# dselivanov/rsparse

Hardware: AMD Instinct MI355X
Metric: als_iterations_per_sec (higher is better)
Workload: dtype f32 (Gram products of rows > 512 / <= 32 non-zeros as 2 x fp16 / 3 x bf16 split terms of the fp32 operands, fp32 accumulate; everything else fp32); 1 GPU; WRMF implicit ALS, CG(3), synthetic 10000000x1000000, 500155883 nnz, rank 128, lambda 0.1; survey_config=3, feedback=implicit, n_items=1000000, nnz=500155883, rank=128, solver=conjugate_gradient, cg_steps=3, parallelism=rows sharded x1, factors replicated

## Files before the change

### rsparse_amd/csrc/wrmf_cgq.hip

```cpp
#include <algorithm>

#include "wrmf_internal.h"
#include "wrmf_device.h"

namespace rsparse_hip {
namespace {

using namespace dev;

constexpr int kGvFirstMinCapq = 16;
constexpr int kStreamPrefixQ = 4;
constexpr int kIdxPrefetchMaxWpr = 2;

constexpr int kMaxSavedSweeps = 4;

template <int KP>
struct QG {
  static constexpr int RPN = KP / 16;
  static constexpr int VW = RPN >= 4 ? 4 : RPN;
  static constexpr int NV = RPN / VW;
  __device__ static __forceinline__ int elem(int i, int r) { return (r / VW) * (16 * VW) + i * VW + (r % VW); }
};

template <int VW>
struct Piece;
template <>
struct Piece<4> { using type = float4; };
template <>
struct Piece<2> { using type = float2; };

__device__ __forceinline__ float groups_reduce_scatter4(const float a0, const float a1, const float a2, const float a3) {
  const auto s01 = __builtin_amdgcn_permlane16_swap(__float_as_uint(a0), __float_as_uint(a1), false, false);
  const float c = __uint_as_float(s01[0]) + __uint_as_float(s01[1]);
  const auto s23 = __builtin_amdgcn_permlane16_swap(__float_as_uint(a2), __float_as_uint(a3), false, false);
  const float d = __uint_as_float(s23[0]) + __uint_as_float(s23[1]);
  const auto t = __builtin_amdgcn_permlane32_swap(__float_as_uint(c), __float_as_uint(d), false, false);
  return __uint_as_float(t[0]) + __uint_as_float(t[1]);
}
template <int KP, int CAPQ, int WAVES, int WPR, int STREAM, bool IMPLICIT, int DMF = 0>
struct QSmem {
  static constexpr size_t gram_floats = (IMPLICIT && DMF != 1) ? (size_t)KP * KP : 0;
  static constexpr size_t vec_floats = IMPLICIT ? (size_t)WAVES * KP : 0;
  static constexpr size_t red_floats = WPR > 1 ? (size_t)2 * WAVES * KP + 2 * WAVES : 0;
  static constexpr bool cv_lds = !STREAM && CAPQ * (KP / 16) > 128;
  static constexpr bool wideq = !STREAM && CAPQ * (KP / 16) > 160;
  static constexpr size_t tsv_floats = (STREAM && !IMPLICIT) ? 0 : (size_t)WAVES * (cv_lds ? 3 : 2) * CAPQ * 4;
  static constexpr size_t pre_floats = STREAM ? (size_t)WAVES * kStreamPrefixQ * 4 * KP : 0;
  static constexpr int dmf_ps = KP + 8, dmf_os = KP + 4;
  static constexpr size_t dmf_floats = DMF ? (size_t)WAVES * dmf_ps + (size_t)WAVES * dmf_os : 0;
  static constexpr size_t pfx_floats =
      (!STREAM && WPR > kIdxPrefetchMaxWpr && (CAPQ == 16 || CAPQ == 20 || CAPQ == 24)) ? (size_t)WAVES * 2 * CAPQ * 4 : 0;
  static constexpr size_t wl_floats = cv_lds ? (size_t)WAVES * 2 : 0;
  static constexpr size_t xs_floats = cv_lds ? (size_t)WAVES * KP : 0;
  static constexpr size_t bytes =
      (gram_floats + vec_floats + red_floats + tsv_floats + pre_floats + dmf_floats + pfx_floats + wl_floats + xs_floats) * 4 + 16;
};

constexpr int kLastFull = 0, kLastDotsInLoop = 1, kLastDotsBehind = 2;
struct LastStepChoice { int kp, capq, waves, wpr, stream; bool implicit; int dmf; bool gb, kfull; int form; };
constexpr LastStepChoice kLastStepChoices[] = {
    {64, 32, 4, 1, 0, true, 0, true, false, kLastFull},
    {64, 16, 4, 1, 0, true, 0, true, true, kLastFull},
    {64, 32, 4, 1, 0, true, 0, false, true, kLastFull},
    {64, 16, 4, 1, 0, true, 0, false, false, kLastFull},
    {64, 16, 4, 1, 0, false, 0, false, true, kLastFull},
    {128, 16, 8, 8, 0, true, 0, true, true, kLastFull},
    {128, 16, 8, 8, 0, true, 0, true, false, kLastFull},
    {128, 16, 4, 2, 0, true, 0, true, true, kLastFull},
    {128, 16, 4, 1, 0, true, 2, true, true, kLastFull},
    {128, 16, 8, 8, 0, true, 0, false, false, kLastFull},
    {32, 8, 4, 1, 0, false, 0, false, true, kLastDotsBehind},
    {64, 32, 4, 2, 0, true, 0, true, false, kLastDotsBehind},
    {64, 32, 4, 2, 0, true, 0, false, false, kLastDotsBehind},
    {128, 16, 4, 4, 0, true, 0, true, false, kLastDotsBehind},
    {128, 16, 4, 2, 0, true, 0, true, false, kLastDotsBehind},
    {128, 24, 4, 4, 0, true, 0, false, true, kLastDotsBehind},
    {128, 24, 4, 4, 0, true, 0, false, false, kLastDotsBehind},
    {128, 20, 4, 4, 0, true, 0, false, true, kLastDotsBehind},
    {128, 20, 4, 4, 0, true, 0, false, false, kLastDotsBehind},
    {128, 16, 4, 4, 0, true, 0, false, false, kLastDotsBehind},
    {128, 16, 4, 2, 0, true, 0, false, false, kLastDotsBehind},
    {128, 16, 4, 1, 0, true, 2, false, false, kLastDotsBehind},
    {128, 20, 4, 4, 0, false, 0, false, true, kLastDotsBehind},
};
constexpr int last_step_form(int KP, int CAPQ, int WAVES, int WPR, int STREAM, bool IMPLICIT, int DMF, bool GB, bool KFULL) {
  for (const LastStepChoice& c : kLastStepChoices)
    if (c.kp == KP && c.capq == CAPQ && c.waves == WAVES && c.wpr == WPR && c.stream == STREAM && c.implicit == IMPLICIT &&
        c.dmf == DMF && c.gb == GB && c.kfull == KFULL)
      return c.form;
  return kLastDotsInLoop;
}

template <int KP, int CAPQ, int WAVES, int WPR, int STREAM, bool IMPLICIT, int DMF = 0, bool GB = false, bool KFULL = false>
__global__ __launch_bounds__(WAVES * 64, 2) void als_cgq_kernel(AlsArgs a, const int32_t* __restrict__ rows, int n_rows,
                                                             int rows_per_team, size_t loss_slot0) {
  using G_ = QG<KP>;
  constexpr int RPN = G_::RPN, VW = G_::VW, NV = G_::NV, CAP = CAPQ * 4, TEAMS = WAVES / WPR;
  using piece_t = typename Piece<VW>::type;
  using SM = QSmem<KP, CAPQ, WAVES, WPR, STREAM, IMPLICIT, DMF>;
  static_assert(WAVES % WPR == 0, "teams must tile the workgroup");
  constexpr bool GRS = RPN == 8 && VW == 4;
  auto groups_all_reduce8 = [](float(&a8)[RPN]) {
    if constexpr (RPN == 8) {
      const float r0 = groups_reduce_scatter4(a8[0], a8[1], a8[2], a8[3]);
      const float r1 = groups_reduce_scatter4(a8[4], a8[5], a8[6], a8[7]);
      float g0[4], g1[4];
      rows_to_all<4>(r0, g0);
      rows_to_all<4>(r1, g1);
#pragma unroll
      for (int e = 0; e < 4; e++) a8[e] = g0[e], a8[4 + e] = g1[e];
    }
  };
  static_assert(!DMF || (IMPLICIT && KP == 128 && WAVES == 4 && WPR == 1 && STREAM == 0), "DMF geometry");
  static_assert(DMF != 1 || CAPQ == 8, "register-resident G terms: only the 8-quad kernel has the 64 registers");
  static_assert(!GB || IMPLICIT, "the global bias of explicit feedback is removed from the data (R/model_WRMF.R:278-282)");
  const float gbias = GB ? a.gbias : 0.f, ltgt = GB ? a.loss_tgt_const : 1.f;
  extern __shared__ __attribute__((aligned(16))) char smem[];
  float* sG = reinterpret_cast<float*>(smem);
  float* sVec = sG + SM::gram_floats;
  float* sRed = sVec + SM::vec_floats;
  float* sRedL = sRed + (WPR > 1 ? 2 * WAVES * KP : 0);
  float* sTsv = sVec + SM::vec_floats + SM::red_floats;
  float* sPre = sTsv + SM::tsv_floats;
  float* sPfx = sPre + SM::pre_floats;
  _Float16* sPh = reinterpret_cast<_Float16*>(sPre + SM::pre_floats);
  _Float16* sPl = sPh + WAVES * SM::dmf_ps;
  float* sOut = reinterpret_cast<float*>(sPl + WAVES * SM::dmf_ps);

  const int tid = threadIdx.x, lane = tid & 63, wv = rfl(tid >> 6);
  const int g = lane >> 4, i = lane & 15;
  const int team = wv / WPR, tw = wv % WPR;
  const int k = KFULL ? KP : a.k;
  if constexpr (IMPLICIT && DMF == 0) {
    constexpr int GU = (KP * KP) % (8 * WAVES * 64) == 0 ? 8 : ((KP * KP) % (2 * WAVES * 64) == 0 ? 2 : 1);
    static_assert((KP * KP) % (GU * WAVES * 64) == 0, "the Gramian copy walks whole batches");
    for (int e0 = tid; e0 < KP * KP; e0 += GU * WAVES * 64) {
      float gv[GU];
#pragma unroll
      for (int u = 0; u < GU; u++) {
        const int e = e0 + u * WAVES * 64, r = e / KP, c = e % KP;
        gv[u] = a.XtX[(size_t)min(r, k - 1) * k + min(c, k - 1)];
      }
#pragma unroll
      for (int u = 0; u < GU; u++) {
        const int e = e0 + u * WAVES * 64, r = e / KP, c = e % KP;
        sG[e] = (r < k && c < k) ? gv[u] : 0.f;
      }
    }
  }
  for (int e = tid; e < (int)(SM::vec_floats + SM::red_floats + SM::tsv_floats); e += WAVES * 64) sVec[e] = 0.f;
  __syncthreads();

  constexpr int NRES = (IMPLICIT && CAPQ == 8 && WPR == 1 && !STREAM && KP == 128 && !DMF) ? 2 : 0;
  piece_t gres[NRES > 0 ? NRES : 1][4][NV];
  if constexpr (NRES > 0) {
#pragma unroll
    for (int rs = 0; rs < NRES; rs++)
#pragma unroll
      for (int u = 0; u < 4; u++)
#pragma unroll
        for (int b = 0; b < NV; b++)
          gres[rs][u][b] = *reinterpret_cast<const piece_t*>(sG + (4 * (g + 4 * rs) + u) * KP + b * 16 * VW + i * VW);
  }
  f16x8 gAh[DMF == 1 ? 2 : 1][DMF == 1 ? 4 : 1], gAl[DMF == 1 ? 2 : 1][DMF == 1 ? 4 : 1];
  char* sGf = reinterpret_cast<char*>(sG) + (size_t)wv * 16 * 1024;
  float ginv = 1.f;
  if constexpr (DMF) {
    const int m = lane & 15, kb = lane >> 4;
    float gmax = 0.f;
#pragma unroll
    for (int t = 0; t < 2; t++)
#pragma unroll
      for (int ks = 0; ks < 4; ks++)
#pragma unroll
        for (int e = 0; e < 8; e++) {
          const int r = 32 * wv + 16 * t + m, c = 32 * ks + 8 * kb + e;
          {
            const float gv = a.XtX[(size_t)min(r, k - 1) * k + min(c, k - 1)];
            gmax = fmaxf(gmax, fabsf(gv) * ((r < k && c < k) ? 1.f : 0.f));
          }
        }
    for (int o = 32; o > 0; o >>= 1) gmax = fmaxf(gmax, __shfl_xor(gmax, o));
    const int ge = fp16_scale_exp(gmax);
    const float gs = __uint_as_float((unsigned)ge << 23);
    ginv = __uint_as_float((unsigned)(254 - ge) << 23);
#pragma unroll
    for (int t = 0; t < 2; t++)
#pragma unroll
      for (int ks = 0; ks < 4; ks++) {
        unsigned hi[4], lo[4];
#pragma unroll
        for (int e = 0; e < 8; e += 2) {
          const int r = 32 * wv + 16 * t + m, c = 32 * ks + 8 * kb + e;
          const float g0v = a.XtX[(size_t)min(r, k - 1) * k + min(c, k - 1)];
          const float g0 = g0v * ((r < k && c < k) ? 1.f : 0.f);
          const float g1v = a.XtX[(size_t)min(r, k - 1) * k + min(c + 1, k - 1)];
          const float g1 = g1v * ((r < k && c + 1 < k) ? 1.f : 0.f);
          split_f16(g0 * gs, g1 * gs, hi[e / 2], lo[e / 2]);
        }
        const uint4 h4 = {hi[0], hi[1], hi[2], hi[3]}, l4 = {lo[0], lo[1], lo[2], lo[3]};
        if constexpr (DMF == 1) {
          gAh[t][ks] = __builtin_bit_cast(f16x8, h4);
          gAl[t][ks] = __builtin_bit_cast(f16x8, l4);
        } else {
          *reinterpret_cast<uint4*>(sGf + ((t * 4 + ks) * 2 + 0) * 1024 + lane * 16) = h4;
          *reinterpret_cast<uint4*>(sGf + ((t * 4 + ks) * 2 + 1) * 1024 + lane * 16) = l4;
        }
      }
    if constexpr (DMF == 2) wave_sync();
  }
  float* vec = sVec + wv * KP;
  constexpr bool CVLDS = SM::cv_lds;
  constexpr bool WIDEQ = SM::wideq;
  float* tacc = sTsv + wv * (CVLDS ? 3 : 2) * CAP;
  float* tcur = tacc + CAP;
  float* csv = tcur + CAP;
  int buf = 0;
  double wloss = 0.0;
  double* wl_lds = reinterpret_cast<double*>(sPfx + SM::pfx_floats) + wv;
  if (CVLDS && lane == 0) *wl_lds = 0.0;
  float* xs = sPfx + SM::pfx_floats + SM::wl_floats + wv * KP;
  int pf_id = 0, pf_cnt = -1;
  float pf_c = 0.f;
  const int team_global = blockIdx.x * TEAMS + team;
  const int total_teams = gridDim.x * TEAMS;

  auto row_index = [&](int itn) { return team_global + itn * total_teams; };
  int row_c = 0, p1_c = 0, p2_c = 0, row_n = 0;
  if (rows_per_team > 0 && row_index(0) < n_rows) {
    row_c = rows[row_index(0)];
    p1_c = a.col_ptrs[row_c];
    p2_c = a.col_ptrs[row_c + 1];
  }
  if (rows_per_team > 1 && row_index(1) < n_rows) row_n = rows[row_index(1)];
  for (int it = 0; it < rows_per_team; ++it) {
    const int ri = row_index(it);
    const bool have = ri < n_rows;
    if (WPR == 1 && !DMF && !have) break;
    const int row = have ? rfl(row_c) : 0;
    const int p1 = have ? rfl(p1_c) : 0;
    const int p2 = have ? rfl(p2_c) : 0;
    constexpr bool META_LATE = WIDEQ && !KFULL;
#define RSP_ADVANCE_META()                                                      \
    {                                                                           \
      int p1_n = 0, p2_n = 0, row_nn = 0;                                       \
      if (it + 1 < rows_per_team && row_index(it + 1) < n_rows) {               \
        p1_n = a.col_ptrs[row_n];                                               \
        p2_n = a.col_ptrs[row_n + 1];                                           \
      }                                                                         \
      if (it + 2 < rows_per_team && row_index(it + 2) < n_rows) row_nn = rows[row_index(it + 2)]; \
      row_c = row_n;                                                            \
      p1_c = p1_n;                                                              \
      p2_c = p2_n;                                                              \
      row_n = row_nn;                                                           \
    }
    if constexpr (!META_LATE) RSP_ADVANCE_META()
    const int cnt = p2 - p1;
    float* yrow = a.Y + (size_t)row * k;
    if (!GB && WPR == 1 && cnt <= 0) {
      if (!DMF || have)
        for (int e = lane; e < k; e += 64) yrow[e] = 0.f;
      if constexpr (!DMF) continue;
    }
    constexpr int PQ = STREAM ? kStreamPrefixQ : 0, PCAP = PQ * 4, PTEAM = PCAP * WPR;
    const int pre = STREAM ? min(cnt, PTEAM) : 0;
    const int pw = STREAM ? max(0, min(PCAP, pre - tw * PCAP)) : 0;
    const int nchunks = (cnt - pre + CAP - 1) / CAP;
    constexpr bool resident = STREAM == 0;
    const float lam_use =
        IMPLICIT ? 0.f : (float)(a.lambda_loss * (a.dynamic_lambda ? (double)(float)cnt : 1.0));

    float* tscr = nullptr;
    float alph[kMaxSavedSweeps];
#pragma unroll
    for (int s2 = 0; s2 < kMaxSavedSweeps; s2++) alph[s2] = 0.f;
    if constexpr (STREAM == 1) {
      if (a.tscr && have && a.cg_steps <= kMaxSavedSweeps) tscr = a.tscr + a.stream_off[ri];
    }

    float xt[CAPQ][RPN];
    float cv[CVLDS ? 1 : CAPQ];
    constexpr int NSL = (CAP + 63) / 64;
    float cl[CVLDS ? 1 : NSL];
#pragma unroll
    for (int s2 = 0; s2 < (CVLDS ? 1 : NSL); s2++) cl[s2] = 0.f;
    auto csv_fill = [&](auto&& conf_of, const int n) {
      const int ln = opaque_lane<WIDEQ>(lane);
#pragma unroll
      for (int s2 = 0; s2 < NSL; s2++) {
        const int sl = ln + 64 * s2;
        if (s2 == 0 || sl < CAP) csv[(sl & 3) * CAPQ + (sl >> 2)] = sl < n ? conf_of(sl) : 0.f;
      }
    };
    int ccnt = 0;

    constexpr bool ZPAD = STREAM == 0;
    constexpr bool TSAVE = STREAM == 0;
    constexpr bool GVFIRST = STREAM == 0 && CAPQ >= kGvFirstMinCapq;
    constexpr bool IDXPF = CAP <= 64 && ((STREAM == 0 && WPR <= kIdxPrefetchMaxWpr) || (STREAM == 1 && IMPLICIT));
    constexpr bool DMAPF = KFULL && !IDXPF && SM::pfx_floats > 0;
    int* pfxI = reinterpret_cast<int*>(sPfx) + wv * 2 * CAP;
    float* pfxC = sPfx + wv * 2 * CAP + CAP;
    auto dma_slot = [&](const int j0, const int n) {
      const int j = j0 + min(lane, n - 1);
      dma4(a.row_idx + j, lds_addr(pfxI));
      dma4(a.vals + j, lds_addr(pfxC));
      if constexpr (CAP > 64) {
        if (lane < CAP - 64) {
          const int j2 = j0 + min(lane + 64, n - 1);
          dma4(a.row_idx + j2, lds_addr(pfxI + 64));
          dma4(a.vals + j2, lds_addr(pfxC + 64));
        }
      }
    };
    int pf_pos = -1;
#define RSP_SLOT_IN(q, n) (SM::wideq ? g < (n) - 4 * (q) : 4 * (q) + g < (n))
#define RSP_SLOT_J(q, n) max(SM::wideq ? min(g, (n) - 1 - 4 * (q)) + 4 * (q) : min(4 * (q) + g, (n) - 1), 0)
    auto gather_q = [&](auto nq_tag, const int base, const int n, const bool from_pf = false) {
      constexpr int NQG = decltype(nq_tag)::value;
      int id[NQG > 0 ? NQG : 1];
      if constexpr (DMAPF) {
        if (!from_pf && n > 0) {
          dma_slot(base, n);
          wait_vm<0>();
        }
        wave_sync();
#pragma unroll
        for (int q = 0; q < NQG; q++) {
          const int j = RSP_SLOT_J(q, n);
          id[q] = pfxI[j];
          if constexpr (!CVLDS) cv[q] = (!ZPAD || RSP_SLOT_IN(q, n)) ? pfxC[j] : 0.f;
        }
        if constexpr (CVLDS) {
          csv_fill([&](int sl) { return pfxC[sl]; }, n);
        } else if constexpr (TSAVE) {
          const int lo = opaque_lane<true>(lane);
#pragma unroll
          for (int s2 = 0; s2 < NSL; s2++) cl[s2] = lane + 64 * s2 < n ? pfxC[min(lo + 64 * s2, CAP - 1)] : 0.f;
        }
        wave_sync();
      } else if (IDXPF && from_pf) {
        int* xi = reinterpret_cast<int*>(tacc);
        wave_sync();
        xi[lane & (CAP - 1)] = pf_id;
        tcur[lane & (CAP - 1)] = pf_c;
        wave_sync();
#pragma unroll
        for (int q = 0; q < NQG; q++) {
          const int j = RSP_SLOT_J(q, n);
          id[q] = xi[j];
          if constexpr (!CVLDS) cv[q] = (!ZPAD || RSP_SLOT_IN(q, n)) ? tcur[j] : 0.f;
        }
        if constexpr (TSAVE) cl[0] = lane < n ? pf_c : 0.f;
        wave_sync();
      } else {
#pragma unroll
        for (int q = 0; q < NQG; q++) {
          const int j = RSP_SLOT_J(q, n);
          id[q] = a.row_idx[base + j];
          if constexpr (!CVLDS) {
            const float c = a.vals[base + j];
            cv[q] = (!ZPAD || RSP_SLOT_IN(q, n)) ? c : 0.f;
          }
        }
        if constexpr (CVLDS) {
          wave_sync();
          csv_fill([&](int sl) { return a.vals[base + sl]; }, n);
          wave_sync();
        } else if constexpr (TSAVE) {
#pragma unroll
          for (int s2 = 0; s2 < NSL; s2++) cl[s2] = lane + 64 * s2 < n ? a.vals[base + lane + 64 * s2] : 0.f;
        }
      }
      const int ig = (SM::wideq && !KFULL) ? (opaque_lane<true>(lane) & 15) : i;
#pragma unroll
      for (int q = 0; q < NQG; q++) {
        const float* src = (!ZPAD || RSP_SLOT_IN(q, n)) ? a.X + (size_t)id[q] * k : a.zero_row;
#pragma unroll
        for (int b = 0; b < NV; b++) {
          const int off = b * 16 * VW + ig * VW;
          if constexpr (KFULL) {
            const piece_t pc = *reinterpret_cast<const piece_t*>(src + off);
            const float* pf = reinterpret_cast<const float*>(&pc);
#pragma unroll
            for (int c = 0; c < VW; c++) xt[q][b * VW + c] = pf[c];
          } else {
            const piece_t pc = *reinterpret_cast<const piece_t*>(src + min(off, k - VW));
            const float* pf = reinterpret_cast<const float*>(&pc);
#pragma unroll
            for (int c = 0; c < VW; c++) xt[q][b * VW + c] = off < k ? pf[c] : 0.f;
          }
        }
      }
    };
#undef RSP_SLOT_IN
#undef RSP_SLOT_J
    auto gather = [&](const int base, const int n, const bool from_pf = false) {
      gather_q(std::integral_constant<int, CAPQ>{}, base, n, from_pf);
    };
    float* pre_lds = sPre + (size_t)wv * PQ * 4 * KP + g * KP;
    auto prefix_chunk = [&](const bool first) {
      if constexpr (PQ > 0) {
        const int base = p1 + tw * PCAP;
        if (first) {
          gather_q(std::integral_constant<int, PQ>{}, base, pw);
#pragma unroll
          for (int q = 0; q < PQ; q++)
#pragma unroll
            for (int b = 0; b < NV; b++) {
              piece_t pc;
              float* pf = reinterpret_cast<float*>(&pc);
#pragma unroll
              for (int c = 0; c < VW; c++) pf[c] = xt[q][b * VW + c];
              *reinterpret_cast<piece_t*>(pre_lds + q * 4 * KP + b * 16 * VW + i * VW) = pc;
            }
        } else {
#pragma unroll
          for (int q = 0; q < PQ; q++) cv[q] = a.vals[base + min(4 * q + g, pw - 1)];
#pragma unroll
          for (int q = 0; q < PQ; q++)
#pragma unroll
            for (int b = 0; b < NV; b++) {
              const piece_t pc = *reinterpret_cast<const piece_t*>(pre_lds + q * 4 * KP + b * 16 * VW + i * VW);
              const float* pf = reinterpret_cast<const float*>(&pc);
#pragma unroll
              for (int c = 0; c < VW; c++) xt[q][b * VW + c] = pf[c];
            }
        }
      }
    };

    float x[RPN], r[RPN], p[RPN], ap[RPN];
    auto load_warm_start = [&]() {
#pragma unroll
      for (int b = 0; b < NV; b++) {
        const int off = b * 16 * VW + i * VW;
        piece_t pc;
        float* pf = reinterpret_cast<float*>(&pc);
#pragma unroll
        for (int c = 0; c < VW; c++) pf[c] = 0.f;
        if (have && off < k) pc = *reinterpret_cast<const piece_t*>(yrow + off);
#pragma unroll
        for (int c = 0; c < VW; c++) x[b * VW + c] = pf[c];
      }
    };
    constexpr bool WS_FIRST = KFULL && resident;
    if constexpr (WS_FIRST) load_warm_start();
    if constexpr (resident) {
      const int per = min(CAP, (((cnt + WPR - 1) / WPR) + 15) & ~15);
      ccnt = max(0, min(per, cnt - tw * per));
      if constexpr (WS_FIRST) {
        gather(ccnt > 0 ? p1 + tw * per : p1, ccnt, ccnt > 0 && pf_cnt == ccnt);
      } else {
        if (ccnt > 0) gather(p1 + tw * per, ccnt, pf_cnt == ccnt);
      }
      pf_cnt = -1;
    }

    if constexpr (!WS_FIRST) load_warm_start();

    auto quad_pass = [&](const float(&v)[RPN], const int mode, float(&acc)[RPN], float& lacc, float* tsave) {
      float* trec = (mode == 0 ? tacc : tcur) + g;
      constexpr int QB = 4;
#pragma unroll
      for (int q0 = 0; q0 < CAPQ; q0 += QB) {
        if (4 * q0 < ccnt) {
          float t[QB];
          f32x2 s2[QB];
#pragma unroll
          for (int u = 0; u < QB; u++) s2[u] = f32x2{0.f, 0.f};
#pragma unroll
          for (int rr = 0; rr < RPN; rr += 2) {
            const f32x2 va = {v[rr], v[rr + 1]};
#pragma unroll
            for (int u = 0; u < QB; u++) {
              const f32x2 xa = {xt[q0 + u][rr], xt[q0 + u][rr + 1]};
              s2[u] = __builtin_elementwise_fma(xa, va, s2[u]);
            }
          }
#pragma unroll
          for (int u = 0; u < QB; u++) t[u] = s2[u].x + s2[u].y;
#pragma unroll
          for (int u = 0; u < QB; u++) t[u] += dpp<0xB1>(t[u]);
#pragma unroll
          for (int u = 0; u < QB; u++) t[u] += dpp<0x4E>(t[u]);
#pragma unroll
          for (int u = 0; u < QB; u++) t[u] += dpp<0x141>(t[u]);
#pragma unroll
          for (int u = 0; u < QB; u++) t[u] += dpp<0x140>(t[u]);
          float cq[QB];
          if constexpr (CVLDS) {
            const float4 c4 = *reinterpret_cast<const float4*>(csv + g * CAPQ + q0);
            cq[0] = c4.x; cq[1] = c4.y; cq[2] = c4.z; cq[3] = c4.w;
          } else {
#pragma unroll
            for (int u = 0; u < QB; u++) cq[u] = cv[q0 + u];
          }
#pragma unroll
          for (int u = 0; u < QB; u++) {
            const int q = q0 + u;
            const bool valid = ZPAD || 4 * q + g < ccnt;
            const float c = cq[u];
            if constexpr (STREAM == 1) {
              if (tsave && valid && i == 0) tsave[4 * q + g] = t[u];
            } else if constexpr (TSAVE) {
              trec[4 * q] = t[u];
            }
            if (mode == 2) {
              const float d = IMPLICIT ? ltgt - t[u] : c - t[u];
              lacc += valid ? (IMPLICIT ? c * d * d : d * d) : 0.f;
            } else if (mode == 3) {
              const float w = IMPLICIT ? (c - 1.f) * t[u] : t[u];
              lacc = fmaf(valid ? w : 0.f, t[u], lacc);
            } else {
              float w;
              if (mode == 0) w = IMPLICIT ? c - (c - 1.f) * (GB ? t[u] + gbias : t[u]) : c - t[u];
              else w = IMPLICIT ? (c - 1.f) * t[u] : t[u];
              w = valid ? w : 0.f;
#pragma unroll
              for (int rr = 0; rr < RPN; rr++) acc[rr] = fmaf(w, xt[q][rr], acc[rr]);
            }
          }
        }
      }
    };

    auto sweep = [&](const float(&v)[RPN], const int mode, float(&out)[RPN], float& loss_out, const bool live,
                     const int sidx = 0) {
      float acc[RPN];
#pragma unroll
      for (int rr = 0; rr < RPN; rr++) acc[rr] = 0.f;
      float lacc = 0.f;
      float dl = 0.f;
      float vinv = 0.f;
      if constexpr (DMF) {
        if (mode != 2) {
          float vmax = 0.f;
#pragma unroll
          for (int rr = 0; rr < RPN; rr++) vmax = fmaxf(vmax, fabsf(v[rr]));
          vmax = row16_max(vmax);
          const int ve = fp16_scale_exp(vmax);
          const float vs = __uint_as_float((unsigned)ve << 23);
          vinv = __uint_as_float((unsigned)(254 - ve) << 23) * (mode == 0 ? -1.f : 1.f);
          if (g < NV) {
            float w4[VW];
#pragma unroll
            for (int c = 0; c < VW; c++) w4[c] = (g == 0 ? v[c] : v[VW + c]) * vs;
            unsigned h0, l0, h1, l1;
            split_f16(w4[0], w4[1], h0, l0);
            split_f16(w4[2], w4[3], h1, l1);
            const int off = wv * SM::dmf_ps + g * 16 * VW + i * VW;
            *reinterpret_cast<uint2*>(sPh + off) = make_uint2(h0, h1);
            *reinterpret_cast<uint2*>(sPl + off) = make_uint2(l0, l1);
          }
          __syncthreads();
          f32x4 d0[2], d1[2];
#pragma unroll
          for (int t = 0; t < 2; t++) d0[t] = d1[t] = f32x4{0.f, 0.f, 0.f, 0.f};
          const int ln = opaque_lane<DMF == 2>(lane);
          const int nb = (ln & 3) * SM::dmf_ps + 8 * (ln >> 4);
#pragma unroll
          for (int ks = 0; ks < 4; ks++) {
            const f16x8 bh = *reinterpret_cast<const f16x8*>(sPh + nb + 32 * ks);
            const f16x8 bl = *reinterpret_cast<const f16x8*>(sPl + nb + 32 * ks);
#pragma unroll
            for (int t = 0; t < 2; t++) {
              f16x8 ah, al;
              if constexpr (DMF == 1) {
                ah = gAh[t][ks];
                al = gAl[t][ks];
              } else {
                ah = *reinterpret_cast<const f16x8*>(sGf + ((t * 4 + ks) * 2 + 0) * 1024 + ln * 16);
                al = *reinterpret_cast<const f16x8*>(sGf + ((t * 4 + ks) * 2 + 1) * 1024 + ln * 16);
              }
              d0[t] = __builtin_amdgcn_mfma_f32_16x16x32_f16(ah, bh, d0[t], 0, 0, 0);
              d1[t] = __builtin_amdgcn_mfma_f32_16x16x32_f16(ah, bl, d1[t], 0, 0, 0);
              d1[t] = __builtin_amdgcn_mfma_f32_16x16x32_f16(al, bh, d1[t], 0, 0, 0);
            }
          }
          if ((ln & 15) < 4) {
#pragma unroll
            for (int t = 0; t < 2; t++) {
              const f32x4 d = (d0[t] + d1[t]) * ginv;
              *reinterpret_cast<f32x4*>(sOut + (ln & 15) * SM::dmf_os + 32 * wv + 16 * t + 4 * (ln >> 4)) = d;
            }
          }
        }
      }
      if (live) {
        if constexpr (IMPLICIT && !DMF) {
          if (mode != 2) {
            wave_sync();
            if (g == 0) {
#pragma unroll
              for (int b = 0; b < NV; b++) {
                piece_t pc;
                float* pf = reinterpret_cast<float*>(&pc);
#pragma unroll
                for (int c = 0; c < VW; c++) pf[c] = v[b * VW + c];
                *reinterpret_cast<piece_t*>(vec + b * 16 * VW + i * VW) = pc;
              }
            }
            wave_sync();
          }
        }
        auto dense_part = [&]() {
          if (IMPLICIT && !DMF && mode != 2) {
            const float sign = mode == 0 ? -1.f : 1.f;
            if constexpr (NRES > 0) {
#pragma unroll
              for (int rs = 0; rs < NRES; rs++) {
                const int kk = 4 * (g + 4 * rs);
                const float4 vb = *reinterpret_cast<const float4*>(vec + kk);
                const float vv[4] = {sign * vb.x, sign * vb.y, sign * vb.z, sign * vb.w};
#pragma unroll
                for (int u = 0; u < 4; u++)
#pragma unroll
                  for (int b = 0; b < NV; b++) {
                    const float* pf = reinterpret_cast<const float*>(&gres[rs][u][b]);
#pragma unroll
                    for (int c = 0; c < VW; c++) acc[b * VW + c] = fmaf(vv[u], pf[c], acc[b * VW + c]);
                  }
              }
            }
            for (int s4 = tw * 4 + g + 4 * NRES; s4 < KP / 4; s4 += WPR * 4) {
              const int kk = 4 * s4;
              const float4 vb = *reinterpret_cast<const float4*>(vec + kk);
              const float vv[4] = {sign * vb.x, sign * vb.y, sign * vb.z, sign * vb.w};
#pragma unroll
              for (int u = 0; u < 4; u++) {
                const float* grow = sG + (kk + u) * KP;
#pragma unroll
                for (int b = 0; b < NV; b++) {
                  const piece_t pc = *reinterpret_cast<const piece_t*>(grow + b * 16 * VW + i * VW);
                  const float* pf = reinterpret_cast<const float*>(&pc);
#pragma unroll
                  for (int c = 0; c < VW; c++) acc[b * VW + c] = fmaf(vv[u], pf[c], acc[b * VW + c]);
                }
              }
            }
          }
        };
        if constexpr (GVFIRST) {
          dense_part();
          if (mode == 3) {
#pragma unroll
            for (int rr = 0; rr < RPN; rr++) dl = fmaf(acc[rr], v[rr], dl);
          }
        }
        if (resident) {
          if (mode != 2 || !TSAVE) {
            quad_pass(v, mode, acc, lacc, nullptr);
          } else {
            wave_sync();
            float esum = 0.f;
            const int ln = opaque_lane<WIDEQ>(lane);
#pragma unroll
            for (int s2 = 0; s2 < NSL; s2++) {
              const int sl = NSL == 1 ? (lane & (CAP - 1)) : min(ln + 64 * s2, CAP - 1);
              const float t = tacc[sl];
              const float clv = CVLDS ? csv[(sl & 3) * CAPQ + (sl >> 2)] : cl[s2];
              const float d = IMPLICIT ? ltgt - t : clv - t;
              const float e = IMPLICIT ? clv * d * d : d * d;
              esum += ln + 64 * s2 < ccnt ? e : 0.f;
            }
            lacc = row16_sum(esum);
          }
        } else if (mode == 2 && tscr) {
          for (int ch = tw; ch < (cnt + CAP - 1) / CAP; ch += WPR) {
            const int n = min(CAP, cnt - ch * CAP);
            if (lane < n) {
              const size_t pos = (size_t)ch * CAP + lane;
              float t = tscr[pos];
#pragma unroll
              for (int s2 = 0; s2 < kMaxSavedSweeps; s2++)
                if (s2 < a.cg_steps && alph[s2] != 0.f) t = fmaf(alph[s2], tscr[(size_t)(s2 + 1) * a.stream_nnz + pos], t);
              const float c = a.vals[p1 + pos];
              const float d = IMPLICIT ? ltgt - t : c - t;
              lacc += IMPLICIT ? c * d * d : d * d;
            }
          }
          lacc = row16_sum(lacc);
        } else {
          if (pw > 0) {
            prefix_chunk(mode == 0);
            ccnt = pw;
            quad_pass(v, mode, acc, lacc, tscr ? tscr + (size_t)sidx * a.stream_nnz + (size_t)tw * PCAP : nullptr);
          }
          for (int ch = tw; ch < nchunks; ch += WPR) {
            ccnt = min(CAP, cnt - pre - ch * CAP);
            gather(p1 + pre + ch * CAP, ccnt, IDXPF && pf_pos == ch && pf_cnt == ccnt);
            if constexpr (IDXPF) {
              const int nch = ch + WPR < nchunks ? ch + WPR : tw;
              const int ncc = min(CAP, cnt - pre - nch * CAP);
              const int j = p1 + pre + nch * CAP + min(lane & (CAP - 1), ncc - 1);
              pf_id = a.row_idx[j];
              pf_c = a.vals[j];
              pf_cnt = ncc;
              pf_pos = nch;
            }
            quad_pass(v, mode, acc, lacc,
                      tscr ? tscr + (size_t)sidx * a.stream_nnz + (size_t)pre + (size_t)ch * CAP : nullptr);
          }
        }
        if constexpr (!GVFIRST) {
          dense_part();
          if (mode == 3) {
#pragma unroll
            for (int rr = 0; rr < RPN; rr++) dl = fmaf(acc[rr], v[rr], dl);
          }
        }
        if constexpr (!DMF) {
          if (mode == 3) {
            if constexpr (IMPLICIT) lacc += row16_sum(dl);
            lacc = groups_sum(lacc);
          } else if (mode != 2) {
            if constexpr (GRS) {
              if constexpr (WPR == 1) groups_all_reduce8(acc);
            } else {
#pragma unroll
              for (int rr = 0; rr < RPN; rr++) acc[rr] = groups_sum(acc[rr]);
            }
          } else {
            lacc = groups_sum(lacc);
          }
        }
      }
      if constexpr (DMF) {
        if (mode != 2) {
          __syncthreads();
          const float f = g == 0 ? vinv : 0.f;
#pragma unroll
          for (int b = 0; b < NV; b++) {
            const f32x4 o = *reinterpret_cast<const f32x4*>(sOut + wv * SM::dmf_os + b * 16 * VW + i * VW);
#pragma unroll
            for (int c = 0; c < VW; c++) {
              if (mode == 3) dl = fmaf(o[c], v[b * VW + c], dl);
              else acc[b * VW + c] = fmaf(f, o[c], acc[b * VW + c]);
            }
          }
          if (mode == 3) {
            lacc = groups_sum(fmaf(f, row16_sum(dl), lacc));
          } else if constexpr (GRS) {
            groups_all_reduce8(acc);
          } else {
#pragma unroll
            for (int rr = 0; rr < RPN; rr++) acc[rr] = groups_sum(acc[rr]);
          }
        } else {
          lacc = groups_sum(lacc);
        }
      }
      if constexpr (WPR > 1) {
        float* red = sRed + buf * WAVES * KP;
        if (mode < 2) {
          if constexpr (GRS) {
            const float r0 = groups_reduce_scatter4(acc[0], acc[1], acc[2], acc[3]);
            const float r1 = groups_reduce_scatter4(acc[4], acc[5], acc[6], acc[7]);
            red[wv * KP + 4 * i + g] = r0;
            red[wv * KP + 64 + 4 * i + g] = r1;
          } else if (g == 0) {
#pragma unroll
            for (int b = 0; b < NV; b++) {
              piece_t pc;
              float* pf = reinterpret_cast<float*>(&pc);
#pragma unroll
              for (int c = 0; c < VW; c++) pf[c] = acc[b * VW + c];
              *reinterpret_cast<piece_t*>(red + wv * KP + b * 16 * VW + i * VW) = pc;
            }
          }
        } else if (lane == 0) {
          sRedL[buf * WAVES + wv] = lacc;
        }
        __syncthreads();
        if (mode < 2) {
#pragma unroll
          for (int rr = 0; rr < RPN; rr++) acc[rr] = 0.f;
#pragma unroll
          for (int w2 = 0; w2 < WPR; w2++) {
#pragma unroll
            for (int b = 0; b < NV; b++) {
              const piece_t pc = *reinterpret_cast<const piece_t*>(red + (team * WPR + w2) * KP + b * 16 * VW + i * VW);
              const float* pf = reinterpret_cast<const float*>(&pc);
#pragma unroll
              for (int c = 0; c < VW; c++) acc[b * VW + c] += pf[c];
            }
          }
        } else {
          lacc = 0.f;
#pragma unroll
          for (int w2 = 0; w2 < WPR; w2++) lacc += sRedL[buf * WAVES + team * WPR + w2];
        }
        buf ^= 1;
      } else {
        __builtin_amdgcn_sched_barrier(0);
      }
      if (mode < 2) {
#pragma unroll
        for (int rr = 0; rr < RPN; rr++) out[rr] = acc[rr];
        if constexpr (GB) {
          if (mode == 0) {
#pragma unroll
            for (int b = 0; b < NV; b++) {
              const int off = b * 16 * VW + i * VW;
              const piece_t pc = *reinterpret_cast<const piece_t*>(a.rhs_init + min(off, k - VW));
              const float* pf = reinterpret_cast<const float*>(&pc);
#pragma unroll
              for (int c = 0; c < VW; c++) out[b * VW + c] += off < k ? pf[c] : 0.f;
            }
          }
        }
        if constexpr (!IMPLICIT) {
#pragma unroll
          for (int rr = 0; rr < RPN; rr++) out[rr] = fmaf(mode == 0 ? -lam_use : lam_use, v[rr], out[rr]);
        }
      } else {
        if constexpr (!IMPLICIT) {
          if (mode == 3) {
            float vv = 0.f;
#pragma unroll
            for (int rr = 0; rr < RPN; rr++) vv = fmaf(v[rr], v[rr], vv);
            lacc = fmaf(lam_use, row16_sum(vv), lacc);
          }
        }
        loss_out = lacc;
      }
    };

    auto dot16 = [&](const float(&u)[RPN], const float(&w)[RPN]) {
      float s = 0.f;
#pragma unroll
      for (int rr = 0; rr < RPN; rr++) s = fmaf(u[rr], w[rr], s);
      return row16_sum(s);
    };

    const bool live = have && (GB || cnt > 0);
    float dummy = 0.f;
    sweep(x, 0, r, dummy, live);
    auto x_piece = [&](const int b) { return reinterpret_cast<piece_t*>(xs + b * 16 * VW + i * VW); };
    if constexpr (CVLDS) {
      if (g == 0) {
#pragma unroll
        for (int b = 0; b < NV; b++) {
          piece_t pc;
          float* pf = reinterpret_cast<float*>(&pc);
#pragma unroll
          for (int c = 0; c < VW; c++) pf[c] = x[b * VW + c];
          *x_piece(b) = pc;
        }
      }
    }
    if constexpr (META_LATE) RSP_ADVANCE_META()
#undef RSP_ADVANCE_META
    if constexpr (IDXPF && STREAM == 0) {
      if (it + 1 < rows_per_team && row_index(it + 1) < n_rows) {
        const int np1 = rfl(p1_c), ncnt = rfl(p2_c) - np1;
        const int nper = min(CAP, (((ncnt + WPR - 1) / WPR) + 15) & ~15);
        const int ncc = max(0, min(nper, ncnt - tw * nper));
        if (ncc > 0) {
          const int j = np1 + tw * nper + min(lane & (CAP - 1), ncc - 1);
          pf_id = a.row_idx[j];
          pf_c = a.vals[j];
          pf_cnt = ncc;
        }
      }
    }
    if constexpr (DMAPF) {
      if (it + 1 < rows_per_team && row_index(it + 1) < n_rows) {
        const int np1 = rfl(p1_c), ncnt = rfl(p2_c) - np1;
        const int nper = min(CAP, (((ncnt + WPR - 1) / WPR) + 15) & ~15);
        const int ncc = max(0, min(nper, ncnt - tw * nper));
        if (ncc > 0) {
          dma_slot(np1 + tw * nper, ncc);
          pf_cnt = ncc;
        }
      }
    }
#pragma unroll
    for (int rr = 0; rr < RPN; rr++) p[rr] = r[rr];
    float rsold = dot16(r, r);
    bool conv = false;
#define RSP_STEP_X(alpha, step)                                                                   \
    do {                                                                                          \
      _Pragma("unroll") for (int s2 = 0; s2 < kMaxSavedSweeps; s2++)                              \
        if (s2 == (step)) alph[s2] = (alpha);                                                     \
      if constexpr (TSAVE) {                                                                      \
        wave_sync();                                                                              \
        const int ln = opaque_lane<WIDEQ>(lane);                                                  \
        _Pragma("unroll") for (int s2 = 0; s2 < NSL; s2++) {                                      \
          const int sl = NSL == 1 ? (lane & (CAP - 1)) : ln + 64 * s2;                            \
          if (CAP % 64 == 0 || sl < CAP) tacc[sl] = fmaf((alpha), tcur[sl], tacc[sl]);            \
        }                                                                                         \
        wave_sync();                                                                              \
      }                                                                                           \
      if constexpr (CVLDS) {                                                                      \
        if (g == 0) {                                                                             \
          _Pragma("unroll") for (int b = 0; b < NV; b++) {                                        \
            piece_t pc = *x_piece(b);                                                             \
            float* pf = reinterpret_cast<float*>(&pc);                                            \
            _Pragma("unroll") for (int c = 0; c < VW; c++) pf[c] = fmaf((alpha), p[b * VW + c], pf[c]); \
            *x_piece(b) = pc;                                                                     \
          }                                                                                       \
        }                                                                                         \
      } else {                                                                                    \
        _Pragma("unroll") for (int rr = 0; rr < RPN; rr++) x[rr] = fmaf((alpha), p[rr], x[rr]);   \
      }                                                                                           \
    } while (0)
#define RSP_LAST_STEP()                                                                           \
    do {                                                                                          \
      float pap = 0.f;                                                                            \
      sweep(p, 3, ap, pap, live && !conv, a.cg_steps);                                            \
      if (!conv) {                                                                                \
        const float alpha = (float)((double)rsold / (double)pap);                                 \
        RSP_STEP_X(alpha, a.cg_steps - 1);                                                        \
      }                                                                                           \
    } while (0)
    constexpr int LAST = last_step_form(KP, CAPQ, WAVES, WPR, STREAM, IMPLICIT, DMF, GB, KFULL);
    for (int itc = 0; itc < a.cg_steps; ++itc) {
      if (WPR == 1 && !DMF && conv) break;
      if (LAST != kLastFull && itc + 1 == a.cg_steps) {
        if constexpr (LAST == kLastDotsInLoop) RSP_LAST_STEP();
        break;
      }
      sweep(p, 1, ap, dummy, live && !conv, itc + 1);
      if (!conv) {
        const float pap = dot16(p, ap);
        const float alpha = (float)((double)rsold / (double)pap);
        RSP_STEP_X(alpha, itc);
#pragma unroll
        for (int rr = 0; rr < RPN; rr++) r[rr] = fmaf(-alpha, ap[rr], r[rr]);
        const float rsnew = dot16(r, r);
        if (rsnew < kCgTol) {
          conv = true;
        } else {
          const float beta = (float)((double)rsnew / (double)rsold);
#pragma unroll
          for (int rr = 0; rr < RPN; rr++) p[rr] = fmaf(p[rr], beta, r[rr]);
          rsold = rsnew;
        }
      }
    }
    if constexpr (LAST == kLastDotsBehind) {
      if (a.cg_steps > 0 && !(WPR == 1 && !DMF && conv)) RSP_LAST_STEP();
    }
#undef RSP_LAST_STEP
#undef RSP_STEP_X
    if constexpr (CVLDS) {
      wave_sync();
#pragma unroll
      for (int b = 0; b < NV; b++) {
        const piece_t pc = *x_piece(b);
        const float* pf = reinterpret_cast<const float*>(&pc);
#pragma unroll
        for (int c = 0; c < VW; c++) x[b * VW + c] = pf[c];
      }
    }
    float rl = 0.f;
    sweep(x, 2, ap, rl, live);
    if constexpr (META_LATE) p1_c = rfl(p1_c), p2_c = rfl(p2_c);
    if constexpr (DMAPF) wait_vm<0>();
    if constexpr (IDXPF && STREAM == 0) {
      asm volatile("" : "+v"(pf_id), "+v"(pf_c));
    }
    if (live && tw == 0) {
      const float xx = dot16(x, x);
      const double wl_row = IMPLICIT ? (double)rl + a.lambda_loss * (double)xx : (double)(rl + lam_use * xx);
      if constexpr (CVLDS) {
        if (lane == 0) *wl_lds += wl_row;
      } else {
        wloss += wl_row;
      }
      if (g == 0) {
#pragma unroll
        for (int b = 0; b < NV; b++) {
          const int off = b * 16 * VW + i * VW;
          if (off < k) {
            piece_t pc;
            float* pf = reinterpret_cast<float*>(&pc);
#pragma unroll
            for (int c = 0; c < VW; c++) pf[c] = x[b * VW + c];
            *reinterpret_cast<piece_t*>(yrow + off) = pc;
          }
        }
      }
    }
  }
  if (lane == 0) a.loss_partials[loss_slot0 + (size_t)blockIdx.x * WAVES + wv] = CVLDS ? *wl_lds : wloss;
}

struct BucketDef { int waves, wpr, capq, stream, max_len; };
constexpr int kNB = 6;
constexpr int kNCfg = 2;
constexpr BucketDef kBuckets[kNCfg][kNB] = {
    {{8, 8, 16, 1, 0x7fffffff}, {8, 8, 16, 0, 512}, {4, 4, 16, 0, 256}, {4, 2, 16, 0, 128}, {4, 1, 16, 0, 64}, {4, 1, 8, 0, 32}},
    {{8, 8, 16, 1, 0x7fffffff}, {4, 4, 32, 0, 512}, {4, 2, 32, 0, 256}, {4, 1, 32, 0, 128}, {4, 1, 16, 0, 64}, {4, 1, 8, 0, 32}},
};
constexpr int cfg_of_kp(int KP) { return KP == 64 ? 1 : 0; }
constexpr int kTeam4Waves = 4, kTeam4Capq = 20;
static_assert(kTeam4Max == kTeam4Waves * kTeam4Capq * 4, "wrmf_internal.h's split and the kernel's capacity");
constexpr int kTeam4WideCapq = 24;
static_assert(kTeam4WideMax == kTeam4Waves * kTeam4WideCapq * 4, "wrmf_schedule.h's split and the wide kernel's capacity");
static_assert(kTeam4Max < kTeam4WideMax && kTeam4WideMax < 512, "the 4-wave launches take bucket 1's rows from its short end");
static_assert(QSmem<128, kTeam4WideCapq, kTeam4Waves, kTeam4Waves, 0, true>::bytes <= 80 * 1024, "the wide team kernel's LDS");
constexpr bool team4_split(int KP, bool GB) { return KP == 128 && !GB; }
int team4_first(const QSchedule& q) { return std::min(std::max(q.team4_first, q.off[1]), q.off[2]); }
int team4_wide_first(const QSchedule& q) { return std::min(std::max(q.team4_wide_first, q.off[1]), team4_first(q)); }

template <int KP, int WAVES, int CAPQ, int WPR, int STREAM, bool IMPLICIT, bool GB, int DMF = 0, bool KFULL = false>
hipError_t launch_bucket(const AlsArgs& a, const int32_t* rows, int n_rows, int grid, size_t slot0, hipStream_t s,
                         hipEvent_t* ev_slot) {
  if (n_rows <= 0) return hipSuccess;
  constexpr bool kDmfGeometry = IMPLICIT && KP == 128 && WAVES == 4 && WPR == 1 && (CAPQ == 8 || CAPQ == 16) && STREAM == 0;
  if constexpr (kDmfGeometry && !DMF) {
    return launch_bucket<KP, WAVES, CAPQ, WPR, STREAM, IMPLICIT, GB, CAPQ == 8 ? 1 : 2>(a, rows, n_rows, grid, slot0, s, ev_slot);
  } else {
    if constexpr (!KFULL && STREAM == 0 && !(DMF == 1 && !GB)) {
      if (a.k == KP)
        return launch_bucket<KP, WAVES, CAPQ, WPR, STREAM, IMPLICIT, GB, DMF, true>(a, rows, n_rows, grid, slot0, s, ev_slot);
    }
    constexpr int TEAMS = WAVES / WPR;
    auto kern = als_cgq_kernel<KP, CAPQ, WAVES, WPR, STREAM, IMPLICIT, DMF, GB, KFULL>;
    const size_t lds = QSmem<KP, CAPQ, WAVES, WPR, STREAM, IMPLICIT, DMF>::bytes;
    hipError_t err = hipFuncSetAttribute(reinterpret_cast<const void*>(kern),
                                         hipFuncAttributeMaxDynamicSharedMemorySize, (int)lds);
    if (err != hipSuccess) return err;
    const int total_teams = grid * TEAMS;
    const int rpt = (n_rows + total_teams - 1) / total_teams;
    prof_note(ev_slot, reinterpret_cast<const void*>(kern));
    hipLaunchKernelGGL(kern, dim3(grid), dim3(WAVES * 64), lds, s, a, rows, n_rows, rpt, slot0);
    return hipGetLastError();
  }
}

struct BucketStreams {
  hipStream_t st[kNB] = {nullptr, nullptr, nullptr, nullptr, nullptr, nullptr};
  hipEvent_t fork = nullptr, fork0 = nullptr;
  hipEvent_t done[kNB] = {nullptr, nullptr, nullptr, nullptr, nullptr, nullptr};
  int device = -1;
  hipError_t ensure() {
    int dev = 0;
    hipError_t err = hipGetDevice(&dev);
    if (err != hipSuccess) return err;
    if (dev == device) return hipSuccess;
    device = dev;
    if ((err = hipEventCreateWithFlags(&fork, hipEventDisableTiming)) != hipSuccess) return err;
    if ((err = hipEventCreateWithFlags(&fork0, hipEventDisableTiming)) != hipSuccess) return err;
    for (int b = 0; b < kNB; b++) {
      if ((err = hipStreamCreateWithFlags(&st[b], hipStreamNonBlocking)) != hipSuccess) return err;
      if ((err = hipEventCreateWithFlags(&done[b], hipEventDisableTiming)) != hipSuccess) return err;
    }
    return hipSuccess;
  }
};
thread_local BucketStreams g_bs;

int g_launch_mode = 2;
int concurrent_buckets() { return g_launch_mode; }

size_t bucket_slots(const QSchedule& q, int b, int k, bool implicit) {
  const int cfg = cfg_of_kp(padded_rank(k));
  const BucketDef d = kBuckets[cfg][b];
  if (d.wpr <= 0) return 0;
  if (d.stream && ne_supported(k)) return (size_t)(q.ne.entries + q.ne.nsplit) + (size_t)(q.mf_n > 0 ? cg_mf_loss_slots(q.mf_n) : 0);
  const int rows = q.off[b + 1] - q.off[b];
  if (b == 1 && padded_rank(k) == 128) {
    const int wide = team4_wide_first(q), split = team4_first(q);
    return (size_t)cgq_bucket_grid(wide - q.off[b], b, cfg) * d.waves + (size_t)cgq_team4_wide_grid(split - wide) * kTeam4Waves +
           (size_t)cgq_team4_grid(q.off[b + 1] - split) * kTeam4Waves;
  }
  if (b == kNB - 1 && rows > 0 && cgp_supported(k, implicit)) {
// ... 187 lines not shown
```

Measured before the change: 8.414 iterations/s.

## Gather next row's factor tiles during last CG step in 8-wave bucket

For the KP=128, 8-wave, 8-waves-per-row, capacity-16 implicit bucket, the next row's index/value slot is double-buffered in LDS. The next row's gathered X tiles and warm start are loaded inside the last CG step's quad pass, so that gather overlaps current-row compute instead of sitting at the start of the next row. It keeps x and the loss accumulator in LDS for this geometry to free registers. The cost is extra LDS, a persistent xt register array and more complex synchronisation, which may lower occupancy.

```diff
diff --git a/rsparse_amd/csrc/wrmf_cgq.hip b/rsparse_amd/csrc/wrmf_cgq.hip
--- a/rsparse_amd/csrc/wrmf_cgq.hip
+++ b/rsparse_amd/csrc/wrmf_cgq.hip
@@ -36,6 +36,11 @@
   const float d = __uint_as_float(s23[0]) + __uint_as_float(s23[1]);
   const auto t = __builtin_amdgcn_permlane32_swap(__float_as_uint(c), __float_as_uint(d), false, false);
   return __uint_as_float(t[0]) + __uint_as_float(t[1]);
+}
+template <bool FIRST, class A, class B>
+__device__ __forceinline__ auto& pick_ref(A& a, B& b) {
+  if constexpr (FIRST) return a;
+  else return b;
 }
 template <int KP, int CAPQ, int WAVES, int WPR, int STREAM, bool IMPLICIT, int DMF = 0>
 struct QSmem {
@@ -48,12 +53,16 @@
   static constexpr size_t pre_floats = STREAM ? (size_t)WAVES * kStreamPrefixQ * 4 * KP : 0;
   static constexpr int dmf_ps = KP + 8, dmf_os = KP + 4;
   static constexpr size_t dmf_floats = DMF ? (size_t)WAVES * dmf_ps + (size_t)WAVES * dmf_os : 0;
+  static constexpr bool early_geom = KP == 128 && CAPQ == 16 && WAVES == 8 && WPR == 8 && !STREAM && IMPLICIT && DMF == 0;
   static constexpr size_t pfx_floats =
-      (!STREAM && WPR > kIdxPrefetchMaxWpr && (CAPQ == 16 || CAPQ == 20 || CAPQ == 24)) ? (size_t)WAVES * 2 * CAPQ * 4 : 0;
-  static constexpr size_t wl_floats = cv_lds ? (size_t)WAVES * 2 : 0;
-  static constexpr size_t xs_floats = cv_lds ? (size_t)WAVES * KP : 0;
+      (!STREAM && WPR > kIdxPrefetchMaxWpr && (CAPQ == 16 || CAPQ == 20 || CAPQ == 24)) ? (size_t)WAVES * 2 * CAPQ * 4 * (early_geom ? 2 : 1) : 0;
+  static constexpr bool x_lds = cv_lds || early_geom;
+  static constexpr size_t wl_floats = x_lds ? (size_t)WAVES * 2 : 0;
+  static constexpr size_t xs_floats = x_lds ? (size_t)WAVES * KP : 0;
+  static constexpr size_t ws_floats = early_geom ? (size_t)WAVES * 256 : 0;
   static constexpr size_t bytes =
-      (gram_floats + vec_floats + red_floats + tsv_floats + pre_floats + dmf_floats + pfx_floats + wl_floats + xs_floats) * 4 + 16;
+      (gram_floats + vec_floats + red_floats + tsv_floats + pre_floats + dmf_floats + pfx_floats + wl_floats + xs_floats + ws_floats) * 4 +
+      16;
 };
 
 constexpr int kLastFull = 0, kLastDotsInLoop = 1, kLastDotsBehind = 2;
@@ -91,6 +100,17 @@
   return kLastDotsInLoop;
 }
 
+struct EarlyGatherChoice { int capq, waves, wpr; };
+constexpr EarlyGatherChoice kEarlyGatherChoices[] = {
+    {16, 8, 8},
+};
+constexpr bool early_gather(int KP, int CAPQ, int WAVES, int WPR, int STREAM, bool IMPLICIT, int DMF, bool GB, bool KFULL) {
+  if (KP != 128 || STREAM != 0 || !IMPLICIT || DMF != 0 || GB || !KFULL) return false;
+  for (const EarlyGatherChoice& c : kEarlyGatherChoices)
+    if (c.capq == CAPQ && c.waves == WAVES && c.wpr == WPR) return true;
+  return false;
+}
+
 template <int KP, int CAPQ, int WAVES, int WPR, int STREAM, bool IMPLICIT, int DMF = 0, bool GB = false, bool KFULL = false>
 __global__ __launch_bounds__(WAVES * 64, 2) void als_cgq_kernel(AlsArgs a, const int32_t* __restrict__ rows, int n_rows,
                                                              int rows_per_team, size_t loss_slot0) {
@@ -211,6 +231,7 @@
   }
   float* vec = sVec + wv * KP;
   constexpr bool CVLDS = SM::cv_lds;
+  constexpr bool XLDS = SM::cv_lds || early_gather(KP, CAPQ, WAVES, WPR, STREAM, IMPLICIT, DMF, GB, KFULL);
   constexpr bool WIDEQ = SM::wideq;
   float* tacc = sTsv + wv * (CVLDS ? 3 : 2) * CAP;
   float* tcur = tacc + CAP;
@@ -218,7 +239,7 @@
   int buf = 0;
   double wloss = 0.0;
   double* wl_lds = reinterpret_cast<double*>(sPfx + SM::pfx_floats) + wv;
-  if (CVLDS && lane == 0) *wl_lds = 0.0;
+  if (XLDS && lane == 0) *wl_lds = 0.0;
   float* xs = sPfx + SM::pfx_floats + SM::wl_floats + wv * KP;
   int pf_id = 0, pf_cnt = -1;
   float pf_c = 0.f;
@@ -233,6 +254,14 @@
     p2_c = a.col_ptrs[row_c + 1];
   }
   if (rows_per_team > 1 && row_index(1) < n_rows) row_n = rows[row_index(1)];
+  constexpr bool EARLY = early_gather(KP, CAPQ, WAVES, WPR, STREAM, IMPLICIT, DMF, GB, KFULL);
+  static_assert(!EARLY || (!CVLDS && SM::early_geom && CAP == 64 && VW == 4 &&
+                           last_step_form(KP, CAPQ, WAVES, WPR, STREAM, IMPLICIT, DMF, GB, KFULL) != kLastFull),
+                "the early gather needs QSmem's room for it (two index slots, x, the next warm start) and the dots-only last step");
+  float xt_keep[EARLY ? CAPQ : 1][RPN];
+  int slot = 0;
+  float* ws = sPfx + SM::pfx_floats + SM::wl_floats + SM::xs_floats + wv * 256;
+  bool eg_done = false;
   for (int it = 0; it < rows_per_team; ++it) {
     const int ri = row_index(it);
     const bool have = ri < n_rows;
@@ -278,8 +307,9 @@
       if (a.tscr && have && a.cg_steps <= kMaxSavedSweeps) tscr = a.tscr + a.stream_off[ri];
     }
 
-    float xt[CAPQ][RPN];
-    float cv[CVLDS ? 1 : CAPQ];
+    float xt_row[EARLY ? 1 : CAPQ][RPN];
+    auto& xt = pick_ref<EARLY>(xt_keep, xt_row);
+    float cv[(CVLDS || EARLY) ? 1 : CAPQ];
     constexpr int NSL = (CAP + 63) / 64;
     float cl[CVLDS ? 1 : NSL];
 #pragma unroll
@@ -293,14 +323,28 @@
       }
     };
     int ccnt = 0;
+    int eg_n = 0;
+    bool eg_pass = false;
 
     constexpr bool ZPAD = STREAM == 0;
     constexpr bool TSAVE = STREAM == 0;
     constexpr bool GVFIRST = STREAM == 0 && CAPQ >= kGvFirstMinCapq;
     constexpr bool IDXPF = CAP <= 64 && ((STREAM == 0 && WPR <= kIdxPrefetchMaxWpr) || (STREAM == 1 && IMPLICIT));
     constexpr bool DMAPF = KFULL && !IDXPF && SM::pfx_floats > 0;
-    int* pfxI = reinterpret_cast<int*>(sPfx) + wv * 2 * CAP;
-    float* pfxC = sPfx + wv * 2 * CAP + CAP;
+    int* pfxI = reinterpret_cast<int*>(sPfx) + wv * 2 * CAP * (EARLY ? 2 : 1) + (EARLY ? slot * 2 * CAP : 0);
+    float* pfxC = reinterpret_cast<float*>(pfxI) + CAP;
+    int* pfnI = reinterpret_cast<int*>(sPfx) + wv * 2 * CAP * (EARLY ? 2 : 1) + (EARLY ? (slot ^ 1) * 2 * CAP : 0);
+    auto dma_slot_e = [&](const int j0, const int n, int* dI) {
+      const int ln = opaque_lane<true>(lane);
+      const int j = j0 + min(4 * (ln & 15) + (ln >> 4), n - 1);
+      dma4(a.row_idx + j, lds_addr(dI));
+      dma4(a.vals + j, lds_addr(dI + CAP));
+    };
+    auto slot_fix = [&](int* dI, const int n) {
+      const int ln = opaque_lane<true>(lane);
+      if (4 * (ln & 15) + (ln >> 4) >= n) reinterpret_cast<float*>(dI)[CAP + ln] = 0.f;
+      wave_sync();
+    };
     auto dma_slot = [&](const int j0, const int n) {
       const int j = j0 + min(lane, n - 1);
       dma4(a.row_idx + j, lds_addr(pfxI));
@@ -319,7 +363,16 @@
     auto gather_q = [&](auto nq_tag, const int base, const int n, const bool from_pf = false) {
       constexpr int NQG = decltype(nq_tag)::value;
       int id[NQG > 0 ? NQG : 1];
-      if constexpr (DMAPF) {
+      if constexpr (EARLY) {
+        if (!from_pf && n > 0) {
+          dma_slot_e(base, n, pfxI);
+          wait_vm<0>();
+        }
+        wave_sync();
+        slot_fix(pfxI, n);
+#pragma unroll
+        for (int q = 0; q < NQG; q++) id[q] = pfxI[g * CAPQ + q];
+      } else if constexpr (DMAPF) {
         if (!from_pf && n > 0) {
           dma_slot(base, n);
           wait_vm<0>();
@@ -445,11 +498,27 @@
       }
     };
     constexpr bool WS_FIRST = KFULL && resident;
-    if constexpr (WS_FIRST) load_warm_start();
+    if constexpr (WS_FIRST && !EARLY) load_warm_start();
     if constexpr (resident) {
       const int per = min(CAP, (((cnt + WPR - 1) / WPR) + 15) & ~15);
       ccnt = max(0, min(per, cnt - tw * per));
-      if constexpr (WS_FIRST) {
+      if constexpr (EARLY) {
+        if (eg_done) {
+          wait_vm<2 * CAPQ>();
+          wave_sync();
+#pragma unroll
+          for (int b = 0; b < NV; b++) {
+            const piece_t pc = *reinterpret_cast<const piece_t*>(ws + b * 16 * VW + i * VW);
+            const float* pf = reinterpret_cast<const float*>(&pc);
+#pragma unroll
+            for (int c = 0; c < VW; c++) x[b * VW + c] = pf[c];
+          }
+        } else {
+          load_warm_start();
+          gather(ccnt > 0 ? p1 + tw * per : p1, ccnt, ccnt > 0 && pf_cnt == ccnt);
+        }
+        eg_done = false;
+      } else if constexpr (WS_FIRST) {
         gather(ccnt > 0 ? p1 + tw * per : p1, ccnt, ccnt > 0 && pf_cnt == ccnt);
       } else {
         if (ccnt > 0) gather(p1 + tw * per, ccnt, pf_cnt == ccnt);
@@ -489,8 +558,8 @@
 #pragma unroll
           for (int u = 0; u < QB; u++) t[u] += dpp<0x140>(t[u]);
           float cq[QB];
-          if constexpr (CVLDS) {
-            const float4 c4 = *reinterpret_cast<const float4*>(csv + g * CAPQ + q0);
+          if constexpr (CVLDS || EARLY) {
+            const float4 c4 = *reinterpret_cast<const float4*>((EARLY ? pfxC : csv) + g * CAPQ + q0);
             cq[0] = c4.x; cq[1] = c4.y; cq[2] = c4.z; cq[3] = c4.w;
           } else {
 #pragma unroll
@@ -519,6 +588,25 @@
               w = valid ? w : 0.f;
 #pragma unroll
               for (int rr = 0; rr < RPN; rr++) acc[rr] = fmaf(w, xt[q][rr], acc[rr]);
+            }
+          }
+        }
+        if constexpr (EARLY) {
+          if (eg_pass) {
+            const int ln = opaque_lane<true>(lane), gg = ln >> 4, io = (ln & 15) * VW;
+            const int4 id4 = *reinterpret_cast<const int4*>(pfnI + gg * CAPQ + q0);
+            const int idn[QB] = {id4.x, id4.y, id4.z, id4.w};
+#pragma unroll
+            for (int u = 0; u < QB; u++) {
+              const int q = q0 + u;
+              const float* src = (gg < eg_n - 4 * q ? a.X + (size_t)idn[u] * k : a.zero_row) + io;
+#pragma unroll
+              for (int b = 0; b < NV; b++) {
+                const piece_t pc = *reinterpret_cast<const piece_t*>(src + b * 16 * VW);
+                const float* pf = reinterpret_cast<const float*>(&pc);
+#pragma unroll
+                for (int c = 0; c < VW; c++) xt[q][b * VW + c] = pf[c];
+              }
             }
           }
         }
@@ -641,16 +729,28 @@
             }
           }
         };
+        bool requesting = false;
+        if constexpr (EARLY) requesting = mode == 3 && eg_n > 0;
         if constexpr (GVFIRST) {
-          dense_part();
-          if (mode == 3) {
-#pragma unroll
-            for (int rr = 0; rr < RPN; rr++) dl = fmaf(acc[rr], v[rr], dl);
+          if (!requesting) {
+            dense_part();
+            if (mode == 3) {
+#pragma unroll
+              for (int rr = 0; rr < RPN; rr++) dl = fmaf(acc[rr], v[rr], dl);
+            }
           }
         }
         if (resident) {
           if (mode != 2 || !TSAVE) {
-            quad_pass(v, mode, acc, lacc, nullptr);
+            if constexpr (!EARLY) {
+              quad_pass(v, mode, acc, lacc, nullptr);
+            } else if (requesting) {
+              eg_pass = true;
+              quad_pass(v, mode, acc, lacc, nullptr);
+              eg_pass = false;
+            } else {
+              quad_pass(v, mode, acc, lacc, nullptr);
+            }
           } else {
             wave_sync();
             float esum = 0.f;
@@ -659,7 +759,7 @@
             for (int s2 = 0; s2 < NSL; s2++) {
               const int sl = NSL == 1 ? (lane & (CAP - 1)) : min(ln + 64 * s2, CAP - 1);
               const float t = tacc[sl];
-              const float clv = CVLDS ? csv[(sl & 3) * CAPQ + (sl >> 2)] : cl[s2];
+              const float clv = (CVLDS || EARLY) ? (EARLY ? pfxC : csv)[(sl & 3) * CAPQ + (sl >> 2)] : cl[s2];
               const float d = IMPLICIT ? ltgt - t : clv - t;
               const float e = IMPLICIT ? clv * d * d : d * d;
               esum += ln + 64 * s2 < ccnt ? e : 0.f;
@@ -709,6 +809,12 @@
 #pragma unroll
             for (int rr = 0; rr < RPN; rr++) dl = fmaf(acc[rr], v[rr], dl);
           }
+        } else if constexpr (EARLY) {
+          if (requesting) {
+            dense_part();
+#pragma unroll
+            for (int rr = 0; rr < RPN; rr++) dl = fmaf(acc[rr], v[rr], dl);
+          }
         }
         if constexpr (!DMF) {
           if (mode == 3) {
@@ -838,7 +944,7 @@
     float dummy = 0.f;
     sweep(x, 0, r, dummy, live);
     auto x_piece = [&](const int b) { return reinterpret_cast<piece_t*>(xs + b * 16 * VW + i * VW); };
-    if constexpr (CVLDS) {
+    if constexpr (XLDS) {
       if (g == 0) {
 #pragma unroll
         for (int b = 0; b < NV; b++) {
@@ -871,7 +977,8 @@
         const int nper = min(CAP, (((ncnt + WPR - 1) / WPR) + 15) & ~15);
         const int ncc = max(0, min(nper, ncnt - tw * nper));
         if (ncc > 0) {
-          dma_slot(np1 + tw * nper, ncc);
+          if constexpr (EARLY) dma_slot_e(np1 + tw * nper, ncc, pfnI);
+          else dma_slot(np1 + tw * nper, ncc);
           pf_cnt = ncc;
         }
       }
@@ -893,7 +1000,7 @@
         }                                                                                         \
         wave_sync();                                                                              \
       }                                                                                           \
-      if constexpr (CVLDS) {                                                                      \
+      if constexpr (XLDS)  {                                                                      \
         if (g == 0) {                                                                             \
           _Pragma("unroll") for (int b = 0; b < NV; b++) {                                        \
             piece_t pc = *x_piece(b);                                                             \
@@ -909,6 +1016,20 @@
 #define RSP_LAST_STEP()                                                                           \
     do {                                                                                          \
       float pap = 0.f;                                                                            \
+      if constexpr (EARLY) {                                                                      \
+         \
+         \
+         \
+        if (live && !conv && pf_cnt > 0) {                                                        \
+          wait_vm<0>();                                                                           \
+          wave_sync();                                                                            \
+          slot_fix(pfnI, pf_cnt);                                                                 \
+          eg_n = pf_cnt;                                                                          \
+          const float* yn = a.Y + (size_t)rfl(row_c) * k;                                         \
+          dma16(yn + (lane & 31) * 4, lds_addr(ws));                                              \
+          eg_done = true;                                                                         \
+        }                                                                                         \
+      }                                                                                           \
       sweep(p, 3, ap, pap, live && !conv, a.cg_steps);                                            \
       if (!conv) {                                                                                \
         const float alpha = (float)((double)rsold / (double)pap);                                 \
@@ -945,7 +1066,7 @@
     }
 #undef RSP_LAST_STEP
 #undef RSP_STEP_X
-    if constexpr (CVLDS) {
+    if constexpr (XLDS) {
       wave_sync();
 #pragma unroll
       for (int b = 0; b < NV; b++) {
@@ -958,14 +1079,16 @@
     float rl = 0.f;
     sweep(x, 2, ap, rl, live);
     if constexpr (META_LATE) p1_c = rfl(p1_c), p2_c = rfl(p2_c);
-    if constexpr (DMAPF) wait_vm<0>();
+    if constexpr (EARLY) {
+      if (!eg_done) wait_vm<0>();
+    } else if constexpr (DMAPF) wait_vm<0>();
     if constexpr (IDXPF && STREAM == 0) {
       asm volatile("" : "+v"(pf_id), "+v"(pf_c));
     }
     if (live && tw == 0) {
       const float xx = dot16(x, x);
       const double wl_row = IMPLICIT ? (double)rl + a.lambda_loss * (double)xx : (double)(rl + lam_use * xx);
-      if constexpr (CVLDS) {
+      if constexpr (XLDS) {
         if (lane == 0) *wl_lds += wl_row;
       } else {
         wloss += wl_row;
@@ -984,8 +1107,9 @@
         }
       }
     }
+    if constexpr (EARLY) slot ^= 1;
   }
-  if (lane == 0) a.loss_partials[loss_slot0 + (size_t)blockIdx.x * WAVES + wv] = CVLDS ? *wl_lds : wloss;
+  if (lane == 0) a.loss_partials[loss_slot0 + (size_t)blockIdx.x * WAVES + wv] = XLDS ? *wl_lds : wloss;
 }
 
 struct BucketDef { int waves, wpr, capq, stream, max_len; };
```

Result: no change. 8.418 iterations/s, median of 2 (+0.0%).
